# humanlongevity/tredparse

Hardware: NVIDIA B200
Metric: loci genotyped/sec (higher is better)
Workload: dtype int16 (SW, DPX s16x2) / f64 (likelihood)

## Files before the change

include/tredsw.h:

```cpp
#ifndef TREDSW_H
#define TREDSW_H

#include <stdint.h>

#ifdef __cplusplus
extern "C" {
#endif

struct _profile;
typedef struct _profile s_profile;

typedef struct {
    uint16_t score1;
    uint16_t score2;
    int32_t ref_begin1;
    int32_t ref_end1;
    int32_t read_begin1;
    int32_t read_end1;
    int32_t ref_end2;
    uint32_t *cigar;
    int32_t cigarLen;
} s_align;

s_profile *ssw_init(const int8_t *read, const int32_t readLen, const int8_t *mat, const int32_t n,
// ... 11 lines not shown
#define TREDSW_ERR_ARG (-2)
#define TREDSW_ERR_UNSUPPORTED (-3)
#define TREDSW_ERR_IO (-4)

#define TREDSW_DEVICE_PTRS 1u
#define TREDSW_DEVICE_INPUTS 64u
#define TREDSW_SCORE2 2u
#define TREDSW_NO_BEGIN 4u
#define TREDSW_CIGAR 8u
#define TREDSW_FORCE_WORD 16u
#define TREDSW_GRID_NO_SURFACE 32u

typedef struct tredsw_ctx tredsw_ctx;

int tredsw_version(void);
int tredsw_device_count(void);
const char *tredsw_last_error(void);

tredsw_ctx *tredsw_create(int device, void *stream);
void tredsw_destroy(tredsw_ctx *ctx);
int tredsw_synchronize(tredsw_ctx *ctx);
int tredsw_sm_count(tredsw_ctx *ctx);
int64_t tredsw_launch_count(tredsw_ctx *ctx);
int tredsw_enable_timing(tredsw_ctx *ctx, int on);
int tredsw_get_timing(tredsw_ctx *ctx, float *ms4);
int tredsw_get_timeline(tredsw_ctx *ctx, float *ms10);
int tredsw_int_pipe_peak(tredsw_ctx *ctx, double *giga_lane_instr_per_s);

enum { TREDSW_TAG_NONE = 0, TREDSW_TAG_FULL = 1, TREDSW_TAG_PREF = 2, TREDSW_TAG_POST = 3,
       TREDSW_TAG_REPT = 4, TREDSW_TAG_HANG = 5,
       TREDSW_TAG_REPT_PAIR = 6  };

int tredsw_align_pairs(tredsw_ctx *ctx, const int8_t *qbuf, const int64_t *qoff, int32_t nq,
                       const int8_t *tbuf, const int64_t *toff, int32_t nt, const int32_t *qidx,
                       const int32_t *tidx, int64_t npairs, const int8_t *mat25, int gap_open,
                       int gap_extend, uint32_t flags, int32_t *out, uint32_t *cigar_out,
                       int32_t cigar_cap);

typedef struct {
    int8_t prefix[32];
    int8_t suffix[32];
    int8_t repeat[32];
    int32_t prefix_len;
    int32_t suffix_len;
    int32_t period;
    int32_t max_units;
// ... 234 lines not shown
```

tredparse_b200/_lib.py:

```python
import ctypes
import os
import threading

import numpy as np

HERE = os.path.dirname(os.path.abspath(__file__))
LIB_PATH = os.path.join(HERE, "libtredsw.so")

DEVICE_PTRS, SCORE2, NO_BEGIN, CIGAR, FORCE_WORD = 1, 2, 4, 8, 16
DEVICE_INPUTS = 64

TAG_NAMES = {0: None, 1: "FULL", 2: "PREF", 3: "POST", 4: "REPT", 5: "HANG"}

EXPORTS = [
    "ssw_init", "init_destroy", "ssw_align", "align_destroy", "cigar_int_to_op", "cigar_int_to_len",
    "tredsw_version", "tredsw_device_count", "tredsw_last_error", "tredsw_create", "tredsw_destroy",
    "tredsw_synchronize", "tredsw_sm_count", "tredsw_launch_count", "tredsw_enable_timing",
    "tredsw_get_timing", "tredsw_get_timeline", "tredsw_int_pipe_peak", "tredsw_align_pairs", "tredsw_classify_reads",
    "tredsw_likelihood_grid", "tredsw_pe_kde", "tredsw_genotype_batch", "tredsw_genotype_batch_ex", "tredsw_pack_reads4", "tredsw_narrow_i16",
    "tredsw_bam_open", "tredsw_bam_close", "tredsw_bam_nref", "tredsw_bam_tid", "tredsw_bam_extract_locus",
    "tredsw_bam_region_depth", "tredsw_bam_read_length", "tredsw_bam_clone", "tredsw_bam_inflate_stats", "tredsw_inflate_raw",
    "tredsw_bam_header_signature",
    "tredsw_ingest_batch_run", "tredsw_ingest_batch_view", "tredsw_ingest_batch_free", "tredsw_ingest_batch_emulate",
    "tredsw_inflate_raw_device_code",
    "tredsw_bam_open_unindexed", "tredsw_ingest_scan_run", "tredsw_ingest_scan_emulate", "tredsw_ingest_scan_stats",
    "tredsw_bam_open_stream", "tredsw_bam_header_text",
]


class TredswError(RuntimeError):
    pass


class Family(ctypes.Structure):
    _fields_ = [("prefix", ctypes.c_int8 * 32), ("suffix", ctypes.c_int8 * 32),
                ("repeat", ctypes.c_int8 * 32), ("prefix_len", ctypes.c_int32),
                ("suffix_len", ctypes.c_int32), ("period", ctypes.c_int32),
                ("max_units", ctypes.c_int32), ("clip", ctypes.c_int32),
                ("reserved", ctypes.c_int32 * 3)]

# ... 39 lines not shown


def load():
    global _lib
    with _lock:
        if _lib is not None:
            return _lib
        if not os.path.exists(LIB_PATH):
            raise TredswError(
                "{} is missing: build it with `python -m tredparse_b200.build` (needs nvcc). "
                "tredparse_b200 has no CPU fallback.".format(LIB_PATH))
        lib = ctypes.CDLL(LIB_PATH)
        lib.tredsw_version.restype = ctypes.c_int
        lib.tredsw_device_count.restype = ctypes.c_int
        lib.tredsw_last_error.restype = ctypes.c_char_p
        lib.tredsw_create.restype = _vp
        lib.tredsw_create.argtypes = [ctypes.c_int, _vp]
        lib.tredsw_destroy.restype = None
        lib.tredsw_destroy.argtypes = [_vp]
        lib.tredsw_synchronize.argtypes = [_vp]
        lib.tredsw_sm_count.argtypes = [_vp]
        lib.tredsw_launch_count.restype = ctypes.c_int64
        lib.tredsw_launch_count.argtypes = [_vp]
        lib.tredsw_enable_timing.argtypes = [_vp, ctypes.c_int]
        lib.tredsw_get_timing.argtypes = [_vp, _vp]
        lib.tredsw_get_timeline.argtypes = [_vp, _vp]
        lib.tredsw_int_pipe_peak.argtypes = [_vp, _vp]
        lib.tredsw_align_pairs.restype = ctypes.c_int
        lib.tredsw_align_pairs.argtypes = [_vp, _vp, _vp, ctypes.c_int32, _vp, _vp, ctypes.c_int32, _vp,
                                           _vp, ctypes.c_int64, _vp, ctypes.c_int, ctypes.c_int,
                                           ctypes.c_uint32, _vp, _vp, ctypes.c_int32]
        lib.tredsw_classify_reads.restype = ctypes.c_int
        lib.tredsw_classify_reads.argtypes = [_vp, _vp, _vp, ctypes.c_int32, _vp, _vp, ctypes.c_int32,
                                              _vp, ctypes.c_int, ctypes.c_int, ctypes.c_uint32, _vp, _vp]
        lib.tredsw_likelihood_grid.restype = ctypes.c_int
        lib.tredsw_likelihood_grid.argtypes = [_vp, _vp, ctypes.c_int32, _vp, ctypes.c_int64, _vp,
                                               ctypes.c_int64, _vp, ctypes.c_int64, _vp, ctypes.c_int64,
                                               _vp, ctypes.c_uint32]
        lib.tredsw_pe_kde.restype = ctypes.c_int
        lib.tredsw_pe_kde.argtypes = [_vp, _vp, _vp, ctypes.c_int32, _vp, ctypes.c_uint32]
        lib.tredsw_pack_reads4.restype = ctypes.c_int
        lib.tredsw_pack_reads4.argtypes = [_vp, ctypes.c_int64, _vp, ctypes.c_int]
        lib.tredsw_narrow_i16.restype = ctypes.c_int
        lib.tredsw_narrow_i16.argtypes = [_vp, ctypes.c_int64, _vp, ctypes.c_int]
        _lib = lib
        return lib
# ... 32 lines not shown

    def close(self):
        if getattr(self, "handle", None):
            self.lib.tredsw_destroy(self.handle)
            self.handle = None

    def __del__(self):
        try:
            self.close()
        except Exception:
            pass

    @property
    def sm_count(self):
        return self.lib.tredsw_sm_count(self.handle)

    def synchronize(self):
        check(self.lib.tredsw_synchronize(self.handle), "tredsw_synchronize")

    @property
    def launches(self):
        return int(self.lib.tredsw_launch_count(self.handle))

    def enable_timing(self, on=True):
        check(self.lib.tredsw_enable_timing(self.handle, int(on)), "tredsw_enable_timing")

    def timing(self):
        ms = (ctypes.c_float * 4)()
        check(self.lib.tredsw_get_timing(self.handle, ms), "tredsw_get_timing")
        return {"sw": ms[0], "grid": ms[1], "kde": ms[2], "total": ms[3]}

    def timeline(self):
        ms = (ctypes.c_float * 10)()
        check(self.lib.tredsw_get_timeline(self.handle, ms), "tredsw_get_timeline")
        names = ("sw0", "sw1", "grid0", "grid1", "kde0", "kde1", "inputs", "final", "start", "copied")
        return {n: ms[i] for i, n in enumerate(names)}

    def int_pipe_peak(self):
        v = ctypes.c_double(0)
        check(self.lib.tredsw_int_pipe_peak(self.handle, ctypes.byref(v)), "tredsw_int_pipe_peak")
        return v.value


_default = {}


# ... 11 lines not shown
```

tredparse_b200/csrc/capi.cu:

```cuda
#include "common.cuh"
#include <stdarg.h>

static thread_local char g_err[512] = "";

void tredsw_set_error(const char *fmt, ...) {
    va_list ap;
    va_start(ap, fmt);
    vsnprintf(g_err, sizeof(g_err), fmt, ap);
    va_end(ap);
}

DeviceToken &tredsw_device_token(int device) {
    static DeviceToken tok[64];
    return tok[(device >= 0 && device < 64) ? device : 0];
}

tredsw_ctx::~tredsw_ctx() {
    cudaSetDevice(device);
    if (done_ev) {
        DeviceToken &t = tredsw_device_token(device);
        std::lock_guard<std::mutex> lock(t.mu);
        if (t.ev == done_ev) { t.ev = nullptr; t.sw_end = nullptr; }
        cudaEventDestroy(done_ev);
        if (sw_end_ev) cudaEventDestroy(sw_end_ev);
    }
    DevBuf *all[] = {&d_q, &d_qoff, &d_t, &d_toff, &d_qidx, &d_tidx, &d_out, &d_cigar, &d_scratch, &d_misc,
                     &d_fam, &d_rfam, &d_stats, &d_work, &d_prob, &d_ipool, &d_dpool, &d_surface, &d_marg,
                     &d_res, &d_counter, &d_tiles, &d_pk, &d_pe16, &d_ftab};
    for (DevBuf *b : all) b->release();
    h_in.release(); h_out.release(); h_tab.release();
    for (int i = 0; i < 10; ++i) if (ev[i]) cudaEventDestroy(ev[i]);
    if (own_stream && stream) cudaStreamDestroy(stream);
}

namespace {
__global__ void __launch_bounds__(256) int_peak_kernel(unsigned *sink, int iters, unsigned seed) {
    unsigned a0 = seed + threadIdx.x, a1 = a0 * 3u, a2 = a0 * 5u, a3 = a0 * 7u, a4 = a0 * 11u, a5 = a0 * 13u,
             a6 = a0 * 17u, a7 = a0 * 19u;
    const unsigned b = 0xfffe0001u, c = 0x00030002u;
#pragma unroll 1
    for (int i = 0; i < iters; ++i) {
#pragma unroll
        for (int k = 0; k < 8; ++k) {
            a0 = __viaddmax_s16x2_relu(a0, b, c); a1 = __viaddmax_s16x2_relu(a1, b, c);
            a2 = __viaddmax_s16x2_relu(a2, b, c); a3 = __viaddmax_s16x2_relu(a3, b, c);
            a4 = __viaddmax_s16x2_relu(a4, b, c); a5 = __viaddmax_s16x2_relu(a5, b, c);
            a6 = __viaddmax_s16x2_relu(a6, b, c); a7 = __viaddmax_s16x2_relu(a7, b, c);
        }
    }
    unsigned r = a0 ^ a1 ^ a2 ^ a3 ^ a4 ^ a5 ^ a6 ^ a7;
    if (r == 0x12345678u) sink[0] = r;
// ... 26 lines not shown
    ctx->sm_count = prop.multiProcessorCount;
    ctx->smem_optin = prop.sharedMemPerBlockOptin;
    if (stream) { ctx->stream = (cudaStream_t)stream; ctx->own_stream = false; }
    else {
        if (cudaStreamCreateWithFlags(&ctx->stream, cudaStreamNonBlocking) != cudaSuccess) {
            tredsw_set_error("cudaStreamCreate failed"); delete ctx; return nullptr;
        }
        ctx->own_stream = true;
    }
    return ctx;
}

void tredsw_destroy(tredsw_ctx *ctx) { delete ctx; }

int tredsw_synchronize(tredsw_ctx *ctx) {
    if (!ctx) return TREDSW_ERR_ARG;
    CUDA_TRY(cudaStreamSynchronize(ctx->stream));
    return TREDSW_OK;
}

int tredsw_sm_count(tredsw_ctx *ctx) { return ctx ? ctx->sm_count : 0; }

int64_t tredsw_launch_count(tredsw_ctx *ctx) { return ctx ? ctx->launches : 0; }

int tredsw_enable_timing(tredsw_ctx *ctx, int on) {
    if (!ctx) return TREDSW_ERR_ARG;
    ctx->timing = on != 0;
    for (int i = 0; i < 10; ++i) ctx->ev_valid[i] = false;
    return TREDSW_OK;
}

int tredsw_get_timing(tredsw_ctx *ctx, float *ms4) {
    if (!ctx || !ms4) return TREDSW_ERR_ARG;
    CUDA_TRY(cudaSetDevice(ctx->device));
    CUDA_TRY(cudaStreamSynchronize(ctx->stream));
    const int pairs[4][2] = {{0, 1}, {2, 3}, {4, 5}, {6, 7}};
    for (int k = 0; k < 4; ++k) {
        ms4[k] = 0.f;
        if (ctx->ev_valid[pairs[k][0]] && ctx->ev_valid[pairs[k][1]])
            CUDA_TRY(cudaEventElapsedTime(&ms4[k], ctx->ev[pairs[k][0]], ctx->ev[pairs[k][1]]));
    }
    return TREDSW_OK;
}

int tredsw_get_timeline(tredsw_ctx *ctx, float *ms10) {
    if (!ctx || !ms10) return TREDSW_ERR_ARG;
// ... 150 lines not shown
```

tredparse_b200/csrc/common.cuh:

```cuda
#pragma once
#include <cuda_runtime.h>
#include <stdint.h>
#include <stdio.h>
#include <string.h>
#include <stdlib.h>
#include <vector>
#include <mutex>

#include "../../include/tredsw.h"

#define TREDSW_VERSION 100

void tredsw_set_error(const char *fmt, ...);

#define CUDA_TRY(expr)                                                                        \
    do {                                                                                      \
        cudaError_t _e = (expr);                                                              \
        if (_e != cudaSuccess) {                                                              \
            tredsw_set_error("%s failed: %s (%s:%d)", #expr, cudaGetErrorString(_e), __FILE__, \
                             __LINE__);                                                       \
            return TREDSW_ERR_CUDA;                                                           \
        }                                                                                     \
    } while (0)

// ... 16 lines not shown
struct PinnedBuf {
    void *p = nullptr;
    size_t cap = 0;
    int ensure(size_t bytes) {
        if (bytes <= cap) return TREDSW_OK;
        if (p) cudaFreeHost(p);
        p = nullptr; cap = 0;
        size_t want = bytes + bytes / 4 + 256;
        CUDA_TRY(cudaHostAlloc(&p, want, cudaHostAllocDefault));
        cap = want;
        return TREDSW_OK;
    }
    void release() { if (p) cudaFreeHost(p); p = nullptr; cap = 0; }
    template <class T> T *as() { return reinterpret_cast<T *>(p); }
};

struct tredsw_ctx {
    int device = 0;
    cudaStream_t stream = nullptr;
    bool own_stream = false;
    int sm_count = 0;
    size_t smem_optin = 0;
    DevBuf d_q, d_qoff, d_t, d_toff, d_qidx, d_tidx, d_out, d_cigar, d_scratch, d_misc, d_fam,
        d_rfam, d_stats, d_work, d_prob, d_ipool, d_dpool, d_surface, d_marg, d_res, d_counter, d_tiles, d_pk, d_pe16, d_ftab;
    PinnedBuf h_in, h_out, h_tab;
    cudaEvent_t done_ev = nullptr, sw_end_ev = nullptr, wait_before_sw = nullptr;
    bool record_sw_end = false;
    std::mutex mu;
    long long launches = 0;
    bool timing = false;
    cudaEvent_t ev[10] = {nullptr, nullptr, nullptr, nullptr, nullptr, nullptr, nullptr, nullptr, nullptr, nullptr};
    bool ev_valid[10] = {false, false, false, false, false, false, false, false, false, false};
    void mark(int i) {
        if (!timing) return;
        if (!ev[i]) cudaEventCreate(&ev[i]);
        cudaEventRecord(ev[i], stream);
        ev_valid[i] = true;
    }
    ~tredsw_ctx();
};

static inline bool dev_ptrs(uint32_t flags) { return (flags & TREDSW_DEVICE_PTRS) != 0; }

struct DeviceToken {
    std::mutex mu;
    cudaEvent_t ev = nullptr;
    cudaEvent_t sw_end = nullptr;
// ... 32 lines not shown
```

tredparse_b200/csrc/sw_family.cu:

```cuda
#include "internal.cuh"
#include "sw_sweep.cuh"
#include <type_traits>
#include <algorithm>
#include <vector>

namespace {

constexpr int FAM_W2 = 16;
constexpr int FLANK = 18;
constexpr int CLASS_BOTH = 0, CLASS_FWD = 1, CLASS_RC = 2, NCLASS = 3;

struct FamilySmem {
    int8_t prefix[32], suffix[32], repeat[32];
    int Lp, Ls, P, U, clip;
};

struct ClassifyParams {
    const int8_t *rbuf; const int64_t *roff;
    const int32_t *order;
    const int32_t *grp_start;
    const int32_t *chunk_start;
    const int32_t *grp_perm;
    const tredsw_family *families;
    int ngroups;
    int go, ge;
    int max_rows;
    int allow_fast;
    int match;
    int max_u;
    uint16_t *score_buf;
    uint32_t *pot_buf;
    uint32_t *gbnd_buf;
    int nslots;
    uint32_t one;
    int32_t *counter;
    int32_t *out;
    unsigned long long *stats;
};

__constant__ int8_t c_fmat25[25];

template <class F>
__device__ __forceinline__ void for_each_base(const int8_t *s, int m, F f) {
    int j = 0;
    const int head = min(m, (int)((16u - (unsigned)(reinterpret_cast<uintptr_t>(s) & 15u)) & 15u));
    for (; j < head; ++j) f(j, (int)s[j]);
    for (; j + 16 <= m; j += 16) {
        const uint4 w = __ldg(reinterpret_cast<const uint4 *>(s + j));
        const uint32_t v[4] = {w.x, w.y, w.z, w.w};
#pragma unroll
        for (int k = 0; k < 16; ++k) f(j + k, (int)(int8_t)((v[k >> 2] >> ((k & 3) * 8)) & 0xffu));
    }
    for (; j < m; ++j) f(j, (int)s[j]);
}


__device__ __forceinline__ int fam_code(const FamilySmem &F, int u, int strand, int n, int i) {
    int k = strand ? (n - 1 - i) : i;
    int c;
    if (k < F.Lp) c = F.prefix[k];
// ... 29 lines not shown
__device__ __forceinline__ int rep_base(const FamilySmem &F, int s, int c) { return s ? comp_code(F.repeat[F.P - 1 - c]) : F.repeat[c]; }
__device__ __forceinline__ int suf_base(const FamilySmem &F, int s, int c) { return s ? comp_code(F.prefix[FLANK - 1 - c]) : F.suffix[c]; }

#define PACKED_CELL(HD, E, S, C, HOUT)                                                        \
    {                                                                                         \
        const uint32_t x_ = HD * one + S;                                                     \
        const uint32_t y_ = __vimax3_s16x2(x_, E, Fv[C]);                                     \
        HOUT = __viaddmax_s16x2_relu(y_, mgo2, mgo2);    \
        HD = Hrow[C];                                                                         \
        Hrow[C] = HOUT;                                                                       \
        E = __viaddmax_s16x2(E, mge2, HOUT);                                                  \
        Fv[C] = __viaddmax_s16x2(Fv[C], mge2, HOUT);                                          \
    }

constexpr int STAB_PAD = 20;

__host__ __device__ constexpr int strip_units(int P) { return P >= 12 ? 1 : 12 / P; }
__host__ __device__ constexpr int instance_period(int P) { return P == 6 ? 3 : P; }

template <int NC, int PER, bool HAS_IN, bool HAS_OUT, bool HOOK>
__device__ __forceinline__ void strip_pass(const uint32_t *stab, const uint8_t *codes, int lane, int m, int rows2,
                                           const uint32_t *bin, uint32_t *bout, const uint32_t *pot,
                                           uint32_t (&seg)[NC / PER], uint32_t (&mu)[NC / PER], uint32_t mgo2,
                                           uint32_t mge2, uint32_t one) {
    constexpr int K = NC / PER;
    static_assert(K * PER == NC, "strip = whole units");
    constexpr int NG = (NC + 3) / 4;
    uint32_t Hrow[NC], Fv[NC], pend[K];
#pragma unroll
    for (int c = 0; c < NC; ++c) { Hrow[c] = 0; Fv[c] = 0; }
#pragma unroll
    for (int u = 0; u < K; ++u) pend[u] = 0;
    uint32_t hin_prev = 0;
    auto code_at = [&](int j) { return j < m ? (int)codes[j * 32 + lane] : PAIR_GHOST; };
    auto row_of = [&](int code) { return reinterpret_cast<const uint4 *>(stab + code * STAB_PAD); };
    const uint4 *rowA = row_of(code_at(0)), *rowB = row_of(code_at(1));
    uint4 gA = rowA[0], gB = rowB[0];
    uint32_t bA = 0, bB = 0, pA = 0, pB = 0, bA2 = 0, bB2 = 0, pA2 = 0, pB2 = 0;
    const int j1 = min(2, rows2 - 2);
    if (HAS_IN) { bA = bin[lane]; bB = bin[32 + lane]; bA2 = bin[j1 * 32 + lane]; bB2 = bin[(j1 + 1) * 32 + lane]; }
    if (HOOK) { pA = pot[lane]; pB = pot[32 + lane]; pA2 = pot[j1 * 32 + lane]; pB2 = pot[(j1 + 1) * 32 + lane]; }
    int codeA2 = code_at(2), codeB2 = code_at(3);
    for (int j = 0; j < rows2; j += 2) {
        uint32_t hinA = 0, eA = 0, hinB = 0, eB = 0;
        if (HAS_IN) {
            hinA = sw_prmt(bA, 0, 0x4140); eA = sw_prmt(bA, 0, 0x4342);
            hinB = sw_prmt(bB, 0, 0x4140); eB = sw_prmt(bB, 0, 0x4342);
// ... 14 lines not shown
        sB[0] = gB.x; sB[1] = gB.y; sB[2] = gB.z; sB[3] = gB.w;
        uint32_t hdA = hin_prev, hdB = hinA;
        hin_prev = hinB;
        uint32_t hA = 0, hB = 0;
#pragma unroll
        for (int s = 0; s <= NC; ++s) {
            if ((s & 3) == 0 && s / 4 + 1 < NG) {
                const uint4 a = rowA[s / 4 + 1];
                sA[s + 4] = a.x; sA[s + 5] = a.y; sA[s + 6] = a.z; sA[s + 7] = a.w;
            }
            if (s >= 1 && ((s - 1) & 3) == 0 && (s - 1) / 4 + 1 < NG) {
                const uint4 b = rowB[(s - 1) / 4 + 1];
                sB[s + 3] = b.x; sB[s + 4] = b.y; sB[s + 5] = b.z; sB[s + 6] = b.w;
            }
            if (s == NC - 4 || (NC < 4 && s == 0)) { gA = rowA2[0]; gB = rowB2[0]; }
            if (s < NC) {
                PACKED_CELL(hdA, eA, sA[s], s, hA)
                const int u = s / PER, i = s % PER;
                if (i == 0) pend[u] = hA; else seg[u] = __vimax3_s16x2(seg[u], pend[u], hA);
                if (HOOK && i == PER - 1) {
                    mu[u] = __viaddmax_s16x2(hdA, potHA, mu[u]);
                    mu[u] = __viaddmax_s16x2(eA, potEA, mu[u]);
                }
                if (HAS_OUT && s == NC - 1) bout[j * 32 + lane] = sw_prmt(hA, eA, 0x6420);
            }
            if (s >= 1) {
                PACKED_CELL(hdB, eB, sB[s - 1], s - 1, hB)
                const int u = (s - 1) / PER, i = (s - 1) % PER;
                if (i == PER - 1) seg[u] = __vimax3_s16x2(seg[u], pend[u], hB); else pend[u] = hB;
                if (HOOK && i == PER - 1) {
                    mu[u] = __viaddmax_s16x2(hdB, potHB, mu[u]);
                    mu[u] = __viaddmax_s16x2(eB, potEB, mu[u]);
                }
                if (HAS_OUT && s - 1 == NC - 1) bout[(j + 1) * 32 + lane] = sw_prmt(hB, eB, 0x6420);
            }
        }
        rowA = rowA2; rowB = rowB2; codeA2 = codeA3; codeB2 = codeB3;
        bA = bA2; bB = bB2; bA2 = bA3; bB2 = bB3; pA = pA2; pB = pB2; pA2 = pA3; pB2 = pB3;
    }
}

template <int NC>
__device__ __forceinline__ void suffix_pass(const uint32_t *stab, const uint8_t *codes, int lane, int m, int rows2,
                                            uint32_t *pot, uint32_t &fresh, uint32_t mgo2, uint32_t mge2) {
    constexpr int NG = (NC + 3) / 4;
    uint32_t Grow[NC], Fv[NC];
#pragma unroll
    for (int c = 0; c < NC; ++c) { Grow[c] = 0; Fv[c] = 0; }
    auto code_at = [&](int r) { const int j = rows2 - 1 - r; return (j >= 0 && j < m) ? (int)codes[j * 32 + lane] : PAIR_GHOST; };
    auto row_of = [&](int code) { return reinterpret_cast<const uint4 *>(stab + code * STAB_PAD); };
    uint32_t f0 = 0, f1 = 0;
#define SUFFIX_CELL(GD, E, S, C, GOUT)                                                        \
    {                                                                                         \
        const uint32_t t_ = __vmaxs2(E, Fv[C]);                                               \
        const uint32_t gh_ = __viaddmax_s16x2_relu(t_, mgo2, GD);   \
        GD = Grow[C];                                                                         \
        GOUT = __vadd2(gh_, S);                                                               \
// ... 79 lines not shown
            uint32_t keyA = 0;
            if (s < NC) {
                PACKED_CELL(hdA, eA, sA[s], s, hA)
                keyA = hA * 256u + rcA;
                if (CAPTURE && s % PER == PER - 1) { capHA |= hA & kmask[s / PER]; capEA |= eA & kmask[s / PER]; }
            }
            if (s >= 1) {
                PACKED_CELL(hdB, eB, sB[s - 1], s - 1, hB)
                const uint32_t keyB = hB * 256u + rcB;
                colkey[s - 1] = __vimax3_u16x2(colkey[s - 1], keyA_prev, keyB);
                if (CAPTURE && (s - 1) % PER == PER - 1) { capHB |= hB & kmask[(s - 1) / PER]; capEB |= eB & kmask[(s - 1) / PER]; }
            }
            keyA_prev = keyA;
        }
        if (CAPTURE) { bout[j * 32] = sw_prmt(capHA, capEA, 0x6420); bout[(j + 1) * 32] = sw_prmt(capHB, capEB, 0x6420); }
    }
}

template <int P>
__device__ __noinline__ void locate_packed(const FamilySmem &F, const SwLut *lut, uint32_t *stab, uint32_t *stab2,
                                           uint32_t *colsel, bool &suffix_table_ready, const uint8_t *codes, int lane,
                                           int m, int m_warp, uint32_t *bnd, const uint32_t *gbnd, int R, int go, int ge,
                                           uint32_t one, int G, int cs, int u, int u_main, int half, int sa, int sb,
                                           int *end_ref, int *end_read, unsigned long long &cells) {
    constexpr int K = strip_units(P);
    constexpr int NC = P * K;
    const uint32_t mgo2 = (uint32_t)((-go) & 0xffff) | ((uint32_t)((-go) & 0xffff) << 16);
    const uint32_t mge2 = (uint32_t)((-ge) & 0xffff) | ((uint32_t)((-ge) & 0xffff) << 16);
    const uint32_t go2 = (uint32_t)go * 0x00010001u;
    const int rows2 = (m_warp + 1) & ~1;
    const int su = G * (u_main > 0 ? u_main : u) - 1;
    const int tstar = su / K, kstar = su % K;
    const int sh = half ? 16 : 0;
    int found_col = -1, found_row = 0;
    {
        {
            const uint32_t *src = gbnd + (size_t)tstar * R * 32 + lane;
            for (int j = 0; j < rows2; ++j) bnd[j * 32 + lane] = src[j * 32];
        }
        uint32_t colkey[NC];
        auto pair_row = [&](int j) { return j < m ? (int)codes[j * 32 + lane] : PAIR_GHOST; };
        strip_locate<NC, P, true>(stab, pair_row, rows2, bnd + lane, bnd + lane, u_main > 0 ? -1 : kstar, colkey,
                                  mgo2, mge2, one);
        if (u_main > 0) {
#pragma unroll
            for (int c = NC - 1; c >= 0; --c) {
                const uint32_t k16 = (colkey[c] >> sh) & 0xffffu;
                if (c / P <= kstar && c / P > kstar - G && (int)(k16 >> 8) == cs) { found_col = FLANK + (tstar * K) * P + c; found_row = 255 - (int)(k16 & 0xffu); }
            }
        }
    }
    __syncwarp();
    cells += (unsigned long long)m * 2ull * (unsigned long long)NC;
    if (__any_sync(0xffffffffu, u_main <= 0 && cs < 0x7fff)) {
        if (!suffix_table_ready) {
            if (lane < FLANK) colsel[lane] = sel2(suf_base(F, sa, lane), suf_base(F, sb, lane));
            __syncwarp();
            build_stab<6>(stab2, lut, lane, FLANK, colsel, go2);
            __syncwarp();
            suffix_table_ready = true;
        }
        uint32_t colkey[FLANK];
        auto own_row = [&](int j) { return j < m ? pair_half(codes[j * 32 + lane], half) : SW_CODE_GHOST; };
        strip_locate<FLANK, FLANK, false>(stab2, own_row, rows2, bnd + lane, nullptr, 0, colkey, mgo2, mge2, one);
        if (u_main <= 0) {
#pragma unroll
            for (int c = FLANK - 1; c >= 0; --c) {
                const uint32_t k16 = (colkey[c] >> sh) & 0xffffu;
                if ((int)(k16 >> 8) == cs) { found_col = FLANK + u * F.P + c; found_row = 255 - (int)(k16 & 0xffu); }
            }
        }
        __syncwarp();
        cells += (unsigned long long)m * 2ull * (unsigned long long)FLANK;
    }
    *end_ref = found_col; *end_read = found_row;
}

template <int P>
__device__ __noinline__ void phase1_packed(const FamilySmem &F, const SwLut *lut, uint32_t *stab, uint32_t *colsel,
                                           const uint8_t *codes, int lane, int m, int m_warp, uint32_t *pot,
                                           uint32_t *gbnd, int R, uint8_t *scores, uint8_t *runs, int go, int ge,
                                           uint32_t one, int G, int sa, int sb, unsigned long long &cells) {
    constexpr int K = strip_units(P);
    constexpr int NC = P * K;
    static_assert(NC <= STAB_PAD && FLANK <= STAB_PAD, "strip wider than the score table");
    const uint32_t mgo2 = (uint32_t)((-go) & 0xffff) | ((uint32_t)((-go) & 0xffff) << 16);
    const uint32_t mge2 = (uint32_t)((-ge) & 0xffff) | ((uint32_t)((-ge) & 0xffff) << 16);
    const uint32_t go2 = (uint32_t)go * 0x00010001u;
    const int rows2 = (m_warp + 1) & ~1;
    if (lane < FLANK) colsel[lane] = sel2(suf_base(F, sa, FLANK - 1 - lane), suf_base(F, sb, FLANK - 1 - lane));
    __syncwarp();
    build_stab<NPAIR>(stab, lut, lane, FLANK, colsel);
    __syncwarp();
    uint32_t fresh = 0;
    suffix_pass<FLANK>(stab, codes, lane, m, rows2, pot, fresh, mgo2, mge2);
    __syncwarp();
    if (lane < FLANK) colsel[lane] = sel2(pre_base(F, sa, lane), pre_base(F, sb, lane));
    __syncwarp();
    build_stab<NPAIR>(stab, lut, lane, FLANK, colsel, go2);
    __syncwarp();
    uint32_t run;
    {
        uint32_t seg0[1] = {0u}, mu0[1] = {0u};
        strip_pass<FLANK, FLANK, false, true, false>(stab, codes, lane, m, rows2, nullptr, gbnd, pot, seg0, mu0, mgo2, mge2, one);
        run = seg0[0];
    }
    __syncwarp();
    for (int c = lane; c < NC; c += 32) colsel[c] = sel2(rep_base(F, sa, c % F.P), rep_base(F, sb, c % F.P));
    __syncwarp();
    build_stab<NPAIR>(stab, lut, lane, NC, colsel, go2);
    __syncwarp();
    int nstrips = 0;
    for (int u0 = 0; u0 < F.U * G; u0 += K, ++nstrips) {
        uint32_t seg[K], mu[K];
#pragma unroll
        for (int u = 0; u < K; ++u) { seg[u] = 0; mu[u] = 0; }
        strip_pass<NC, P, true, true, true>(stab, codes, lane, m, rows2, gbnd + (size_t)nstrips * R * 32,
                                            gbnd + (size_t)(nstrips + 1) * R * 32, pot, seg, mu, mgo2, mge2, one);
#pragma unroll
        for (int u = 0; u < K; ++u) {
            run = __vmaxs2(run, seg[u]);
            const int su = u0 + u + 1;
            if (su % G == 0 && su <= F.U * G) {
                const int ur = su / G - 1;
                const uint32_t best = __vimax3_s16x2(run, mu[u], fresh);
                scores[(2 * ur + 0) * 32 + lane] = (uint8_t)(best & 0xffu);
                scores[(2 * ur + 1) * 32 + lane] = (uint8_t)((best >> 16) & 0xffu);
                runs[(2 * ur + 0) * 32 + lane] = (uint8_t)(run & 0xffu);
                runs[(2 * ur + 1) * 32 + lane] = (uint8_t)((run >> 16) & 0xffu);
            }
        }
    }
    cells += (unsigned long long)m * 2ull * (unsigned long long)(2 * FLANK + nstrips * NC);
}

template <bool FAST>
__global__ void __launch_bounds__(32) classify_kernel(ClassifyParams p) {
    extern __shared__ __align__(16) unsigned char smem_raw[];
    __shared__ SwLut lut;
    __shared__ FamilySmem F;
    __shared__ __align__(16) uint32_t stab[NPAIR * STAB_PAD], stab2[6 * STAB_PAD];
    __shared__ uint32_t colsel[STAB_PAD];
    typedef typename std::conditional<FAST, uint8_t, uint16_t>::type score_t;
    const int lane = threadIdx.x;
    const int R = p.max_rows + 2;
    uint32_t *bnd = reinterpret_cast<uint32_t *>(smem_raw);
    uint8_t *codes = reinterpret_cast<uint8_t *>(bnd + (size_t)R * 32);
    unsigned char *slot = reinterpret_cast<unsigned char *>(p.score_buf) + (size_t)blockIdx.x * (2 * p.max_u) * 32 * sizeof(uint16_t);
    score_t *scores = reinterpret_cast<score_t *>(slot);
    uint8_t *runs = slot + (size_t)(2 * p.max_u) * 32;
    uint32_t *pot = FAST ? bnd : p.pot_buf + (size_t)blockIdx.x * R * 32;
    uint32_t *gbnd = p.gbnd_buf + (size_t)blockIdx.x * (p.nslots + 1) * R * 32;
    const uint32_t one = p.one;
    sw_build_lut(&lut, c_fmat25, lane, 32);
    const int nitems = p.chunk_start[p.ngroups];
    unsigned long long alg = 0, cells1 = 0, cells2 = 0;
    unsigned nal = 0;

    for (;;) {
        __syncwarp();
        int item = 0;
        if (lane == 0) item = atomicAdd(p.counter + (FAST ? 1 : 0), 1);
        item = __shfl_sync(0xffffffffu, item, 0);
        if (item >= nitems) break;
        int lo = 0, hi = p.ngroups;
        while (hi - lo > 1) {
            int mid = (lo + hi) >> 1;
            if (p.chunk_start[mid] <= item) lo = mid; else hi = mid;
        }
        const int grp = p.grp_perm[lo], f = grp / NCLASS, cls = grp % NCLASS;
        {
            const tredsw_family &g = p.families[f];
            F.prefix[lane] = g.prefix[lane]; F.suffix[lane] = g.suffix[lane]; F.repeat[lane] = g.repeat[lane];
            if (lane == 0) { F.Lp = g.prefix_len; F.Ls = g.suffix_len; F.P = g.period; F.U = g.max_units; F.clip = g.clip; }
        }
        __syncwarp();
        const bool fast_shape = p.allow_fast && (F.Lp == FLANK && F.Ls == FLANK && F.P >= 1 && F.P <= 12);
        if (fast_shape != FAST) continue;

        const bool pair = FAST && cls != CLASS_BOTH;
        const int sa = cls == CLASS_RC ? 1 : 0, sb = cls == CLASS_FWD ? 0 : 1;
        const int idx0 = p.grp_start[grp] + (pair ? 64 * (item - p.chunk_start[lo]) + 2 * lane : 32 * (item - p.chunk_start[lo]) + lane);
        int r0 = -1, r1 = -1, m0 = 0, m1 = 0;
        const bool valid0 = idx0 < p.grp_start[grp + 1], valid1 = pair && idx0 + 1 < p.grp_start[grp + 1];
        if (valid0) { r0 = p.order[idx0]; m0 = (int)(p.roff[r0 + 1] - p.roff[r0]); }
        if (valid1) { r1 = p.order[idx0 + 1]; m1 = (int)(p.roff[r1 + 1] - p.roff[r1]); }
        const bool too_long0 = m0 > p.max_rows, too_long1 = m1 > p.max_rows;
        if (too_long0) m0 = 0;
        if (too_long1) m1 = 0;
        auto clampc = [](int c) { return (c < 0 || c > 4) ? 4 : c; };
        const int m_lane = max(m0, m1);
        if (!pair) {
            if (m0 > 0) for_each_base(p.rbuf + p.roff[r0], m0, [&](int j, int c) { codes[j * 32 + lane] = (uint8_t)((FAST ? 7 : 1) * clampc(c)); });
        } else {
            if (m0 > 0) for_each_base(p.rbuf + p.roff[r0], m0, [&](int j, int c) { codes[j * 32 + lane] = (uint8_t)(6 * clampc(c) + SW_CODE_GHOST); });
            for (int j = m0; j < m_lane; ++j) codes[j * 32 + lane] = (uint8_t)PAIR_GHOST;
            if (m1 > 0) for_each_base(p.rbuf + p.roff[r1], m1, [&](int j, int c) { codes[j * 32 + lane] += (uint8_t)(clampc(c) - SW_CODE_GHOST); });
        }
        const int m_warp = __reduce_max_sync(0xffffffffu, m_lane);
        __syncwarp();

        if constexpr (!FAST) {
            phase1_generic(F, &lut, codes, lane, m0, m_warp, bnd, scores, p.go, p.ge, cells1);
        } else {
            switch (instance_period(F.P)) {
#define PCASE(PP) case PP: phase1_packed<PP>(F, &lut, stab, colsel, codes, lane, m_lane, m_warp, pot, gbnd, R, scores, runs, p.go, p.ge, one, F.P / PP, sa, sb, cells1); break;
                PCASE(1) PCASE(2) PCASE(3) PCASE(4) PCASE(5) PCASE(7) PCASE(8) PCASE(9) PCASE(10) PCASE(11) PCASE(12)
#undef PCASE
            }
        }
        __syncwarp();

        bool suffix_table_ready = false;
        for (int h = 0; h < (pair ? 2 : 1); ++h) {
            const bool valid = h ? valid1 : valid0, too_long = h ? too_long1 : too_long0;
            const int r = h ? r1 : r0, m = h ? m1 : m0;
            const int own_strand = h ? sb : sa;
            int tag = TREDSW_TAG_NONE, best_u = 0, best_score = -1, rb = -1, re = -1, qb = -1, qe = -1, best_rank = -1;
            const bool active = valid && m > 0;
            auto pick = [&](int last_score, int last_rank, int &cs, int &cr) {
                cs = -1; cr = -1;
                if (!active) return;
                for (int rank = 0; rank < 2 * F.U; ++rank) {
                    if (pair && (rank & 1) != own_strand) continue;
                    const int sc = scores[(pair ? (rank & ~1) | h : rank) * 32 + lane];
                    const int n = F.Lp + F.Ls + F.P * (rank / 2 + 1);
                    const int min_len = min(m, n) / 2;
                    if (sc < max(min_len, 30)) continue;
                    if (sc > last_score || (sc == last_score && rank <= last_rank)) continue;
                    if (sc > cs) { cs = sc; cr = rank; }
                }
            };
            int cs, cr;
            pick(0x7fffffff, -1, cs, cr);
            const int max_units_eff = F.clip ? (m + F.P - 1) / F.P : F.U;
            auto own_code = [&](int j) { return FAST ? pair_half(codes[j * 32 + lane], h) : (int)codes[j * 32 + lane]; };
            while (__any_sync(0xffffffffu, cr >= 0)) {
                const bool pending = cr >= 0;
                const int u = pending ? cr / 2 + 1 : 1, s = pending ? (cr & 1) : 0;
                const int half = pair ? h : s;
                int fast_end_ref = -1, fast_end_read = 0;
                if constexpr (FAST) {
                    if (FLANK * p.match < 30) {
                        int u_main = 0;
                        if (pending) for (int k = 1; k <= u; ++k) if ((int)runs[(2 * (k - 1) + half) * 32 + lane] == cs) { u_main = k; break; }
                        switch (instance_period(F.P)) {
#define PCASE(PP) case PP: locate_packed<PP>(F, &lut, stab, stab2, colsel, suffix_table_ready, codes, lane, m, m_warp, bnd, gbnd, R, p.go, p.ge, one, F.P / PP, pending ? cs : 0x7fff, u, u_main, half, sa, sb, &fast_end_ref, &fast_end_read, cells2); break;
                            PCASE(1) PCASE(2) PCASE(3) PCASE(4) PCASE(5) PCASE(7) PCASE(8) PCASE(9) PCASE(10) PCASE(11) PCASE(12)
#undef PCASE
                        }
                        if (!pending) fast_end_ref = -1;
                    }
                }
                if (pending) {
                    const int n = F.Lp + F.Ls + F.P * u;
                    auto cc_f = [&](int i) { return fam_code(F, u, s, n, i); };
                    int end_ref = fast_end_ref, end_read = fast_end_read;
                    if (end_ref < 0) {
                        const int drift = sw_max_drift(cs, m, n, p.match, p.go, p.ge);
                        const int need = (cs + p.match - 1) / p.match;
                        sw_sweep<FAM_W2, 1, false>(m, m, n, own_code, cc_f, &lut, bnd + lane, 32, p.go, p.ge, cs, &end_ref, &end_read,
                                                   nullptr, -(m - need) - drift, (n - need) + drift, &cells2);
                    }
                    bool settled = false;
                    if (end_ref >= 0) {
                        const int rdrift = sw_max_drift(cs, end_read + 1, end_ref + 1, p.match, p.go, p.ge);
                        int ci = -1, rj = 0;
                        if (rdrift == 0) {
                            const int lim = min(end_read, end_ref) + 1;
                            int hs = 0;
// ... 30 lines not shown
                o[7] = best_rank;
            }
            if (p.stats && active) {
                unsigned long long sum_n = 0;
                for (int u = 1; u <= F.U; ++u) sum_n += 2ull * (unsigned long long)(F.Lp + F.Ls + F.P * u);
                alg += (unsigned long long)m * sum_n;
                nal += (unsigned)(2 * F.U);
            }
        }
    }
    if (p.stats) {
        unsigned long long c1 = cells1, c2 = cells2, na = nal;
        for (int d = 16; d > 0; d >>= 1) {
            alg += __shfl_down_sync(0xffffffffu, alg, d);
            c1 += __shfl_down_sync(0xffffffffu, c1, d);
            c2 += __shfl_down_sync(0xffffffffu, c2, d);
            na += __shfl_down_sync(0xffffffffu, na, d);
        }
        if (lane == 0) {
            atomicAdd(&p.stats[0], alg); atomicAdd(&p.stats[1], c1); atomicAdd(&p.stats[2], c2);
            atomicAdd(&p.stats[3], na);
        }
    }
}

struct QgramInfo {
    int q;
    int min_score;
    int pair;
};
constexpr int QTAB_WORDS = 256;

__global__ void prefilter_kernel(const int8_t *rbuf, const int64_t *roff, int nreads, const int32_t *read_family,
                                 int nfam, const tredsw_family *families, const uint32_t *qtab, const QgramInfo *qinfo,
                                 int b_minus, int32_t *eff_group, unsigned long long *stats) {
    const int r = blockIdx.x * blockDim.x + threadIdx.x;
    unsigned long long alg = 0; unsigned nal = 0;
    if (r < nreads) {
        int f = read_family[r], cls = CLASS_BOTH;
        if (f < 0 || f >= nfam) f = -1;
        if (f >= 0 && qinfo[f].q > 0) {
            const int q = qinfo[f].q;
            const uint32_t mask = (1u << (2 * q)) - 1u;
            const uint32_t *tab = qtab + (size_t)f * QTAB_WORDS;
            const int8_t *s = rbuf + roff[r];
            const int m = (int)(roff[r + 1] - roff[r]);
// ... 131 lines not shown
    const int max_rows = max_m > 0 ? max_m : 1;
    const size_t rows_alloc = (size_t)max_rows + 2;
    const size_t smem = rows_alloc * 32 * 4 + rows_alloc * 32 + 64;
    size_t static_smem = 0;
    int rc;
    if ((rc = classify_static_smem(&static_smem))) return rc;
    if (smem + static_smem > ctx->smem_optin) {
        tredsw_set_error("reads too long for shared memory (%zu B)", smem + static_smem);
        return TREDSW_ERR_UNSUPPORTED;
    }
    ClassifyParams p{};
    p.rbuf = d_rbuf; p.roff = d_roff; p.families = d_families; p.out = d_out;
    const int ngroups = NCLASS * nfamilies;
    int32_t *w = d_work;
    int32_t *d_count = w, *d_grp_start = w + ngroups, *d_chunk_start = d_grp_start + ngroups + 1,
            *d_cursor = d_chunk_start + ngroups + 1, *d_order = d_cursor + ngroups;
    CUDA_TRY(cudaMemsetAsync(d_count, 0, ngroups * sizeof(int32_t), ctx->stream));
    const int tb = 256, nb = (nreads + tb - 1) / tb;
    p.order = d_order; p.grp_start = d_grp_start; p.chunk_start = d_chunk_start;
    p.ngroups = ngroups; p.go = gap_open; p.ge = gap_extend; p.max_rows = max_rows;
    p.allow_fast = allow_fast ? 1 : 0;
    p.match = max_match > 0 ? max_match : 1;
    p.stats = d_stats;
    const int nitems_bound = nreads / 32 + ngroups + 1;
    int nctas = 0;
    if ((rc = persistent_ctas(ctx, smem, static_smem, need_fast, need_generic, &nctas))) return rc;
    if (nctas > nitems_bound) nctas = nitems_bound;
    const size_t score_bytes = (size_t)nctas * 2 * max_u * 32 * sizeof(uint16_t);
    const size_t pot_bytes = (size_t)nctas * rows_alloc * 32 * sizeof(uint32_t);
    const size_t gbnd_bytes = pot_bytes * (nslots + 1);
    const size_t perm_bytes = (((size_t)ngroups * sizeof(int32_t)) + 15) & ~(size_t)15;
    const size_t qtab_bytes = (size_t)nfamilies * QTAB_WORDS * sizeof(uint32_t);
    const size_t qinfo_bytes = (((size_t)nfamilies * sizeof(QgramInfo)) + 15) & ~(size_t)15;
    const size_t eff_bytes = (((size_t)nreads * sizeof(int32_t)) + 15) & ~(size_t)15;
    if ((rc = ctx->d_scratch.ensure(score_bytes + pot_bytes + gbnd_bytes + 16 + perm_bytes + qtab_bytes + qinfo_bytes + eff_bytes))) return rc;
    p.score_buf = ctx->d_scratch.as<uint16_t>();
    p.pot_buf = reinterpret_cast<uint32_t *>(ctx->d_scratch.as<unsigned char>() + score_bytes);
    p.gbnd_buf = reinterpret_cast<uint32_t *>(ctx->d_scratch.as<unsigned char>() + score_bytes + pot_bytes);
    p.nslots = nslots; p.one = 1u;
    p.counter = reinterpret_cast<int32_t *>(ctx->d_scratch.as<unsigned char>() + score_bytes + pot_bytes + gbnd_bytes);
    p.max_u = max_u;
    int32_t *d_perm = p.counter + 4;
    std::vector<int32_t> h_perm;
    {
        std::vector<int32_t> perm(ngroups);
        int group_size[33] = {0};
// ... 139 lines not shown
```

Measured before the change: 1.796 million.

## Skip remaining repeat strips once strip boundary reaches a fixed point

In the packed period-aware phase-1 Smith-Waterman pass, each strip's output boundary is compared with its input boundary. When the boundary is unchanged across the whole warp, later strips would repeat the same computation, so the loop stops and fills the remaining per-unit scores from the last strip's values. The locate pass clamps its boundary slot to the last strip actually computed. The change also adds per-period skip statistics gathered in shared memory and atomics, plus an env var to disable skipping. This costs a few XORs and a warp vote per strip plus stats atomics, and relies on the fixed-point assumption holding exactly.

```diff
diff --git a/include/tredsw.h b/include/tredsw.h
--- a/include/tredsw.h
+++ b/include/tredsw.h
@@ -57,6 +57,8 @@
 int tredsw_synchronize(tredsw_ctx *ctx);
 int tredsw_sm_count(tredsw_ctx *ctx);
 int64_t tredsw_launch_count(tredsw_ctx *ctx);
+#define TREDSW_STRIP_SKIP_STATS 49
+int tredsw_strip_skip_stats(tredsw_ctx *ctx, int64_t *out);
 int tredsw_enable_timing(tredsw_ctx *ctx, int on);
 int tredsw_get_timing(tredsw_ctx *ctx, float *ms4);
 int tredsw_get_timeline(tredsw_ctx *ctx, float *ms10);
diff --git a/tredparse_b200/_lib.py b/tredparse_b200/_lib.py
--- a/tredparse_b200/_lib.py
+++ b/tredparse_b200/_lib.py
@@ -15,7 +15,7 @@
 EXPORTS = [
     "ssw_init", "init_destroy", "ssw_align", "align_destroy", "cigar_int_to_op", "cigar_int_to_len",
     "tredsw_version", "tredsw_device_count", "tredsw_last_error", "tredsw_create", "tredsw_destroy",
-    "tredsw_synchronize", "tredsw_sm_count", "tredsw_launch_count", "tredsw_enable_timing",
+    "tredsw_synchronize", "tredsw_sm_count", "tredsw_launch_count", "tredsw_strip_skip_stats", "tredsw_enable_timing",
     "tredsw_get_timing", "tredsw_get_timeline", "tredsw_int_pipe_peak", "tredsw_align_pairs", "tredsw_classify_reads",
     "tredsw_likelihood_grid", "tredsw_pe_kde", "tredsw_genotype_batch", "tredsw_genotype_batch_ex", "tredsw_pack_reads4", "tredsw_narrow_i16",
     "tredsw_bam_open", "tredsw_bam_close", "tredsw_bam_nref", "tredsw_bam_tid", "tredsw_bam_extract_locus",
@@ -101,6 +101,8 @@
         lib.tredsw_sm_count.argtypes = [_vp]
         lib.tredsw_launch_count.restype = ctypes.c_int64
         lib.tredsw_launch_count.argtypes = [_vp]
+        lib.tredsw_strip_skip_stats.restype = ctypes.c_int
+        lib.tredsw_strip_skip_stats.argtypes = [_vp, _vp]
         lib.tredsw_enable_timing.argtypes = [_vp, ctypes.c_int]
         lib.tredsw_get_timing.argtypes = [_vp, _vp]
         lib.tredsw_get_timeline.argtypes = [_vp, _vp]
@@ -179,6 +181,14 @@
     def launches(self):
         return int(self.lib.tredsw_launch_count(self.handle))
 
+    def strip_skip_stats(self):
+        a = np.zeros(49, dtype=np.int64)
+        check(self.lib.tredsw_strip_skip_stats(self.handle, ptr(a)), "tredsw_strip_skip_stats")
+        per = a[1:].reshape(12, 4)
+        return {"cells_skipped": int(a[0]),
+                "by_period": {p + 1: dict(zip(("planned", "skipped", "items", "items_no_skip"), map(int, per[p])))
+                              for p in range(12) if per[p, 2]}}
+
     def enable_timing(self, on=True):
         check(self.lib.tredsw_enable_timing(self.handle, int(on)), "tredsw_enable_timing")
 
diff --git a/tredparse_b200/csrc/capi.cu b/tredparse_b200/csrc/capi.cu
--- a/tredparse_b200/csrc/capi.cu
+++ b/tredparse_b200/csrc/capi.cu
@@ -26,7 +26,7 @@
     }
     DevBuf *all[] = {&d_q, &d_qoff, &d_t, &d_toff, &d_qidx, &d_tidx, &d_out, &d_cigar, &d_scratch, &d_misc,
                      &d_fam, &d_rfam, &d_stats, &d_work, &d_prob, &d_ipool, &d_dpool, &d_surface, &d_marg,
-                     &d_res, &d_counter, &d_tiles, &d_pk, &d_pe16, &d_ftab};
+                     &d_res, &d_counter, &d_tiles, &d_pk, &d_pe16, &d_ftab, &d_skip};
     for (DevBuf *b : all) b->release();
     h_in.release(); h_out.release(); h_tab.release();
     for (int i = 0; i < 10; ++i) if (ev[i]) cudaEventDestroy(ev[i]);
@@ -99,6 +99,17 @@
 int tredsw_sm_count(tredsw_ctx *ctx) { return ctx ? ctx->sm_count : 0; }
 
 int64_t tredsw_launch_count(tredsw_ctx *ctx) { return ctx ? ctx->launches : 0; }
+
+int tredsw_strip_skip_stats(tredsw_ctx *ctx, int64_t *out) {
+    if (!ctx || !out) { tredsw_set_error("bad arguments"); return TREDSW_ERR_ARG; }
+    std::lock_guard<std::mutex> lock(ctx->mu);
+    memset(out, 0, TREDSW_STRIP_SKIP_STATS * sizeof(int64_t));
+    if (!ctx->d_skip.p) return TREDSW_OK;
+    CUDA_TRY(cudaSetDevice(ctx->device));
+    CUDA_TRY(cudaMemcpyAsync(out, ctx->d_skip.p, TREDSW_STRIP_SKIP_STATS * sizeof(int64_t), cudaMemcpyDeviceToHost, ctx->stream));
+    CUDA_TRY(cudaStreamSynchronize(ctx->stream));
+    return TREDSW_OK;
+}
 
 int tredsw_enable_timing(tredsw_ctx *ctx, int on) {
     if (!ctx) return TREDSW_ERR_ARG;
diff --git a/tredparse_b200/csrc/common.cuh b/tredparse_b200/csrc/common.cuh
--- a/tredparse_b200/csrc/common.cuh
+++ b/tredparse_b200/csrc/common.cuh
@@ -62,7 +62,8 @@
     int sm_count = 0;
     size_t smem_optin = 0;
     DevBuf d_q, d_qoff, d_t, d_toff, d_qidx, d_tidx, d_out, d_cigar, d_scratch, d_misc, d_fam,
-        d_rfam, d_stats, d_work, d_prob, d_ipool, d_dpool, d_surface, d_marg, d_res, d_counter, d_tiles, d_pk, d_pe16, d_ftab;
+        d_rfam, d_stats, d_work, d_prob, d_ipool, d_dpool, d_surface, d_marg, d_res, d_counter, d_tiles, d_pk, d_pe16, d_ftab,
+        d_skip;
     PinnedBuf h_in, h_out, h_tab;
     cudaEvent_t done_ev = nullptr, sw_end_ev = nullptr, wait_before_sw = nullptr;
     bool record_sw_end = false;
diff --git a/tredparse_b200/csrc/sw_family.cu b/tredparse_b200/csrc/sw_family.cu
--- a/tredparse_b200/csrc/sw_family.cu
+++ b/tredparse_b200/csrc/sw_family.cu
@@ -3,6 +3,9 @@
 #include <type_traits>
 #include <algorithm>
 #include <vector>
+#ifdef TREDSW_DEBUG
+#include <assert.h>
+#endif
 
 namespace {
 
@@ -36,6 +39,8 @@
     int32_t *counter;
     int32_t *out;
     unsigned long long *stats;
+    int strip_skip;
+    unsigned long long *skip_stats;
 };
 
 __constant__ int8_t c_fmat25[25];
@@ -111,7 +116,7 @@
 __device__ __forceinline__ void strip_pass(const uint32_t *stab, const uint8_t *codes, int lane, int m, int rows2,
                                            const uint32_t *bin, uint32_t *bout, const uint32_t *pot,
                                            uint32_t (&seg)[NC / PER], uint32_t (&mu)[NC / PER], uint32_t mgo2,
-                                           uint32_t mge2, uint32_t one) {
+                                           uint32_t mge2, uint32_t one, uint32_t &diff) {
     constexpr int K = NC / PER;
     static_assert(K * PER == NC, "strip = whole units");
     constexpr int NG = (NC + 3) / 4;
@@ -172,7 +177,11 @@
                     mu[u] = __viaddmax_s16x2(hdA, potHA, mu[u]);
                     mu[u] = __viaddmax_s16x2(eA, potEA, mu[u]);
                 }
-                if (HAS_OUT && s == NC - 1) bout[j * 32 + lane] = sw_prmt(hA, eA, 0x6420);
+                if (HAS_OUT && s == NC - 1) {
+                    const uint32_t w = sw_prmt(hA, eA, 0x6420);
+                    bout[j * 32 + lane] = w;
+                    if (HAS_IN) diff |= w ^ bA;
+                }
             }
             if (s >= 1) {
                 PACKED_CELL(hdB, eB, sB[s - 1], s - 1, hB)
@@ -182,7 +191,11 @@
                     mu[u] = __viaddmax_s16x2(hdB, potHB, mu[u]);
                     mu[u] = __viaddmax_s16x2(eB, potEB, mu[u]);
                 }
-                if (HAS_OUT && s - 1 == NC - 1) bout[(j + 1) * 32 + lane] = sw_prmt(hB, eB, 0x6420);
+                if (HAS_OUT && s - 1 == NC - 1) {
+                    const uint32_t w = sw_prmt(hB, eB, 0x6420);
+                    bout[(j + 1) * 32 + lane] = w;
+                    if (HAS_IN) diff |= w ^ bB;
+                }
             }
         }
         rowA = rowA2; rowB = rowB2; codeA2 = codeA3; codeB2 = codeB3;
@@ -308,7 +321,7 @@
                                            uint32_t *colsel, bool &suffix_table_ready, const uint8_t *codes, int lane,
                                            int m, int m_warp, uint32_t *bnd, const uint32_t *gbnd, int R, int go, int ge,
                                            uint32_t one, int G, int cs, int u, int u_main, int half, int sa, int sb,
-                                           int *end_ref, int *end_read, unsigned long long &cells) {
+                                           int last_slot, int *end_ref, int *end_read, unsigned long long &cells) {
     constexpr int K = strip_units(P);
     constexpr int NC = P * K;
     const uint32_t mgo2 = (uint32_t)((-go) & 0xffff) | ((uint32_t)((-go) & 0xffff) << 16);
@@ -317,11 +330,14 @@
     const int rows2 = (m_warp + 1) & ~1;
     const int su = G * (u_main > 0 ? u_main : u) - 1;
     const int tstar = su / K, kstar = su % K;
+#ifdef TREDSW_DEBUG
+    assert(u_main <= 0 || tstar < last_slot);
+#endif
     const int sh = half ? 16 : 0;
     int found_col = -1, found_row = 0;
     {
         {
-            const uint32_t *src = gbnd + (size_t)tstar * R * 32 + lane;
+            const uint32_t *src = gbnd + (size_t)min(tstar, last_slot) * R * 32 + lane;
             for (int j = 0; j < rows2; ++j) bnd[j * 32 + lane] = src[j * 32];
         }
         uint32_t colkey[NC];
@@ -363,10 +379,11 @@
 }
 
 template <int P>
-__device__ __noinline__ void phase1_packed(const FamilySmem &F, const SwLut *lut, uint32_t *stab, uint32_t *colsel,
-                                           const uint8_t *codes, int lane, int m, int m_warp, uint32_t *pot,
-                                           uint32_t *gbnd, int R, uint8_t *scores, uint8_t *runs, int go, int ge,
-                                           uint32_t one, int G, int sa, int sb, unsigned long long &cells) {
+__device__ __noinline__ int phase1_packed(const FamilySmem &F, const SwLut *lut, uint32_t *stab, uint32_t *colsel,
+                                          const uint8_t *codes, int lane, int m, int m_warp, uint32_t *pot,
+                                          uint32_t *gbnd, int R, uint8_t *scores, uint8_t *runs, int go, int ge,
+                                          uint32_t one, int G, int sa, int sb, bool skip, int *planned,
+                                          unsigned long long &cells, unsigned long long &skipped_cells) {
     constexpr int K = strip_units(P);
     constexpr int NC = P * K;
     static_assert(NC <= STAB_PAD && FLANK <= STAB_PAD, "strip wider than the score table");
@@ -387,8 +404,9 @@
     __syncwarp();
     uint32_t run;
     {
-        uint32_t seg0[1] = {0u}, mu0[1] = {0u};
-        strip_pass<FLANK, FLANK, false, true, false>(stab, codes, lane, m, rows2, nullptr, gbnd, pot, seg0, mu0, mgo2, mge2, one);
+        uint32_t seg0[1] = {0u}, mu0[1] = {0u}, unused = 0u;
+        strip_pass<FLANK, FLANK, false, true, false>(stab, codes, lane, m, rows2, nullptr, gbnd, pot, seg0, mu0, mgo2, mge2,
+                                                     one, unused);
         run = seg0[0];
     }
     __syncwarp();
@@ -396,28 +414,42 @@
     __syncwarp();
     build_stab<NPAIR>(stab, lut, lane, NC, colsel, go2);
     __syncwarp();
+    auto put = [&](int su, uint32_t mu_u) {
+        if (su % G == 0 && su <= F.U * G) {
+            const int ur = su / G - 1;
+            const uint32_t best = __vimax3_s16x2(run, mu_u, fresh);
+            scores[(2 * ur + 0) * 32 + lane] = (uint8_t)(best & 0xffu);
+            scores[(2 * ur + 1) * 32 + lane] = (uint8_t)((best >> 16) & 0xffu);
+            runs[(2 * ur + 0) * 32 + lane] = (uint8_t)(run & 0xffu);
+            runs[(2 * ur + 1) * 32 + lane] = (uint8_t)((run >> 16) & 0xffu);
+        }
+    };
+    const int nplan = (F.U * G + K - 1) / K;
     int nstrips = 0;
-    for (int u0 = 0; u0 < F.U * G; u0 += K, ++nstrips) {
-        uint32_t seg[K], mu[K];
+    for (int u0 = 0; u0 < F.U * G; u0 += K) {
+        uint32_t seg[K], mu[K], diff = 0u;
 #pragma unroll
         for (int u = 0; u < K; ++u) { seg[u] = 0; mu[u] = 0; }
         strip_pass<NC, P, true, true, true>(stab, codes, lane, m, rows2, gbnd + (size_t)nstrips * R * 32,
-                                            gbnd + (size_t)(nstrips + 1) * R * 32, pot, seg, mu, mgo2, mge2, one);
+                                            gbnd + (size_t)(nstrips + 1) * R * 32, pot, seg, mu, mgo2, mge2, one, diff);
+        ++nstrips;
 #pragma unroll
         for (int u = 0; u < K; ++u) {
             run = __vmaxs2(run, seg[u]);
-            const int su = u0 + u + 1;
-            if (su % G == 0 && su <= F.U * G) {
-                const int ur = su / G - 1;
-                const uint32_t best = __vimax3_s16x2(run, mu[u], fresh);
-                scores[(2 * ur + 0) * 32 + lane] = (uint8_t)(best & 0xffu);
-                scores[(2 * ur + 1) * 32 + lane] = (uint8_t)((best >> 16) & 0xffu);
-                runs[(2 * ur + 0) * 32 + lane] = (uint8_t)(run & 0xffu);
-                runs[(2 * ur + 1) * 32 + lane] = (uint8_t)((run >> 16) & 0xffu);
-            }
-        }
-    }
-    cells += (unsigned long long)m * 2ull * (unsigned long long)(2 * FLANK + nstrips * NC);
+            put(u0 + u + 1, mu[u]);
+        }
+        if (skip && __all_sync(0xffffffffu, diff == 0u)) {
+            for (int v0 = u0 + K; v0 < F.U * G; v0 += K) {
+#pragma unroll
+                for (int u = 0; u < K; ++u) put(v0 + u + 1, mu[u]);
+            }
+            break;
+        }
+    }
+    cells += (unsigned long long)m * 2ull * (unsigned long long)(2 * FLANK + nplan * NC);
+    skipped_cells += (unsigned long long)m * 2ull * (unsigned long long)((nplan - nstrips) * NC);
+    *planned = nplan;
+    return nstrips;
 }
 
 template <bool FAST>
@@ -438,9 +470,11 @@
     uint32_t *pot = FAST ? bnd : p.pot_buf + (size_t)blockIdx.x * R * 32;
     uint32_t *gbnd = p.gbnd_buf + (size_t)blockIdx.x * (p.nslots + 1) * R * 32;
     const uint32_t one = p.one;
+    __shared__ unsigned long long skip_acc[TREDSW_STRIP_SKIP_STATS];
+    for (int i = lane; i < TREDSW_STRIP_SKIP_STATS; i += 32) skip_acc[i] = 0ull;
     sw_build_lut(&lut, c_fmat25, lane, 32);
     const int nitems = p.chunk_start[p.ngroups];
-    unsigned long long alg = 0, cells1 = 0, cells2 = 0;
+    unsigned long long alg = 0, cells1 = 0, cells2 = 0, cells_skipped = 0;
     unsigned nal = 0;
 
     for (;;) {
@@ -486,13 +520,21 @@
         const int m_warp = __reduce_max_sync(0xffffffffu, m_lane);
         __syncwarp();
 
+        int last_slot = 0;
         if constexpr (!FAST) {
             phase1_generic(F, &lut, codes, lane, m0, m_warp, bnd, scores, p.go, p.ge, cells1);
         } else {
-            switch (instance_period(F.P)) {
-#define PCASE(PP) case PP: phase1_packed<PP>(F, &lut, stab, colsel, codes, lane, m_lane, m_warp, pot, gbnd, R, scores, runs, p.go, p.ge, one, F.P / PP, sa, sb, cells1); break;
+            const int pi = instance_period(F.P);
+            int planned = 0;
+            switch (pi) {
+#define PCASE(PP) case PP: last_slot = phase1_packed<PP>(F, &lut, stab, colsel, codes, lane, m_lane, m_warp, pot, gbnd, R, scores, runs, p.go, p.ge, one, F.P / PP, sa, sb, p.strip_skip != 0, &planned, cells1, cells_skipped); break;
                 PCASE(1) PCASE(2) PCASE(3) PCASE(4) PCASE(5) PCASE(7) PCASE(8) PCASE(9) PCASE(10) PCASE(11) PCASE(12)
 #undef PCASE
+            }
+            if (lane == 0) {
+                unsigned long long *a = skip_acc + 1 + 4 * (pi - 1);
+                a[0] += (unsigned long long)planned; a[1] += (unsigned long long)(planned - last_slot);
+                a[2] += 1ull; a[3] += last_slot == planned ? 1ull : 0ull;
             }
         }
         __syncwarp();
@@ -531,7 +573,7 @@
                         int u_main = 0;
                         if (pending) for (int k = 1; k <= u; ++k) if ((int)runs[(2 * (k - 1) + half) * 32 + lane] == cs) { u_main = k; break; }
                         switch (instance_period(F.P)) {
-#define PCASE(PP) case PP: locate_packed<PP>(F, &lut, stab, stab2, colsel, suffix_table_ready, codes, lane, m, m_warp, bnd, gbnd, R, p.go, p.ge, one, F.P / PP, pending ? cs : 0x7fff, u, u_main, half, sa, sb, &fast_end_ref, &fast_end_read, cells2); break;
+#define PCASE(PP) case PP: locate_packed<PP>(F, &lut, stab, stab2, colsel, suffix_table_ready, codes, lane, m, m_warp, bnd, gbnd, R, p.go, p.ge, one, F.P / PP, pending ? cs : 0x7fff, u, u_main, half, sa, sb, last_slot, &fast_end_ref, &fast_end_read, cells2); break;
                             PCASE(1) PCASE(2) PCASE(3) PCASE(4) PCASE(5) PCASE(7) PCASE(8) PCASE(9) PCASE(10) PCASE(11) PCASE(12)
 #undef PCASE
                         }
@@ -608,6 +650,13 @@
             atomicAdd(&p.stats[3], na);
         }
     }
+    if (FAST) {
+        for (int d = 16; d > 0; d >>= 1) cells_skipped += __shfl_down_sync(0xffffffffu, cells_skipped, d);
+        if (lane == 0) skip_acc[0] = cells_skipped;
+        __syncwarp();
+        for (int i = lane; i < TREDSW_STRIP_SKIP_STATS; i += 32)
+            if (skip_acc[i]) atomicAdd(&p.skip_stats[i], skip_acc[i]);
+    }
 }
 
 struct QgramInfo {
@@ -785,6 +834,12 @@
     p.allow_fast = allow_fast ? 1 : 0;
     p.match = max_match > 0 ? max_match : 1;
     p.stats = d_stats;
+    p.strip_skip = getenv("TREDSW_NO_STRIP_SKIP") == nullptr ? 1 : 0;
+    if (!ctx->d_skip.p) {
+        if ((rc = ctx->d_skip.ensure(TREDSW_STRIP_SKIP_STATS * sizeof(unsigned long long)))) return rc;
+        CUDA_TRY(cudaMemsetAsync(ctx->d_skip.p, 0, TREDSW_STRIP_SKIP_STATS * sizeof(unsigned long long), ctx->stream));
+    }
+    p.skip_stats = ctx->d_skip.as<unsigned long long>();
     const int nitems_bound = nreads / 32 + ngroups + 1;
     int nctas = 0;
     if ((rc = persistent_ctas(ctx, smem, static_smem, need_fast, need_generic, &nctas))) return rc;
```

Measured after the change: 1.884 million, median of 6. 4.9% higher.
